# HBioquant/DiffBindFR

Measured on AMD Instinct MI355X. Metric: poses_per_sec, higher is better.
Workload: dtype f32

## Files before the change

### diffbindfr_amd/csrc/convz.hip

```cpp
#include <cstdio>
#include <cstdlib>
#include <type_traits>

#include "common.h"

typedef float f32x4 __attribute__((ext_vector_type(4)));
typedef float f32x2 __attribute__((ext_vector_type(2)));
typedef _Float16 f16x8 __attribute__((ext_vector_type(8)));
typedef _Float16 f16x4 __attribute__((ext_vector_type(4)));
typedef _Float16 f16x2 __attribute__((ext_vector_type(2)));
typedef unsigned u32x4 __attribute__((ext_vector_type(4)));
typedef unsigned u32x2 __attribute__((ext_vector_type(2)));

#define CH_TILE_BYTES 9280
#define CH_TAIL_OFF 8192
#define CH_BIAS_OFF 9216

#define CZ_VSTRIDE 2064
#define CZ_CB (8 * CZ_VSTRIDE)
#define CZ_NCB 2
#define CZ_TILE (CZ_NCB * CZ_CB)
#define CZ_KPB 1
#define CZ_BUF (CZ_KPB * CZ_TILE)
#define CZ_ZBYTES (2 * CZ_BUF)
#define CZ_NHL 2
#define CZ_WAVE_FLOATS (32 * 12 + 32 + 32 + 32 + 32 + 32 + CZ_MAXSEG * 16 + 24 * 64 + CZ_NHL * 256)
#ifndef CZ_PRIO
#define CZ_PRIO 1
#endif
#if CZ_PRIO
#define CZ_SETPRIO(x) __builtin_amdgcn_s_setprio(x)
#else
#define CZ_SETPRIO(x)
#endif
#ifndef CZ_FETCH_AT
#define CZ_FETCH_AT 4
#endif
#ifndef CZ_PF_KT
#define CZ_PF_KT 7
#endif
#define CZ_ZSCALE (-20)

__device__ __forceinline__ void cz_split2(float x0, float x1, unsigned& hi, unsigned& lo) {
  const f16x2 h = __builtin_convertvector((f32x2){x0, x1}, f16x2);
  const f16x2 l = __builtin_convertvector((f32x2){x0 - (float)h[0], x1 - (float)h[1]}, f16x2);
  hi = __builtin_bit_cast(unsigned, h);
  lo = __builtin_bit_cast(unsigned, l);
}
__device__ __forceinline__ float cz_wave_max(float v) {
#pragma unroll
  for (int o = 1; o < 64; o <<= 1) v = fmaxf(v, __shfl_xor(v, o));
  return v;
}

__device__ __forceinline__ int cz_lane_here() {
  int l = __builtin_amdgcn_mbcnt_hi(~0u, __builtin_amdgcn_mbcnt_lo(~0u, 0u));
  asm volatile("" : "+v"(l));
  return l;
}

template <int I, int N, typename F>
__device__ __forceinline__ void cz_static_for(F&& f) {
  if constexpr (I < N) { f(std::integral_constant<int, I>{}); cz_static_for<I + 1, N>(f); }
}

template <int NW, int ABL = 0>
__global__ __launch_bounds__(64 * NW, 2) void k_convz(ConvZArgs a) {
  constexpr int KT = 9;
  extern __shared__ __attribute__((aligned(16))) float lds[];
  const int tid = threadIdx.x, lane = tid & 63, wave = __builtin_amdgcn_readfirstlane(tid >> 6);
  const int n = lane & 15, g = lane >> 4;
  char* zb = reinterpret_cast<char*>(lds);
  float* wl = lds + CZ_ZBYTES / 4 + wave * CZ_WAVE_FLOATS;
  float* w_sh = wl;
  float* w_sa = wl + 32 * 12;
  float* w_ua = w_sa + 32;
  int* w_row = reinterpret_cast<int*>(w_ua + 32);
  int* w_seg = w_row + 32;
  int* w_first = w_seg + 32;
  unsigned* w_mask = reinterpret_cast<unsigned*>(w_first + 32);
  float* w_xs = reinterpret_cast<float*>(w_mask + CZ_MAXSEG * 16);
  u32x4* w_hl = reinterpret_cast<u32x4*>(w_xs + 24 * 64);
  int* b_nseg = reinterpret_cast<int*>(lds + CZ_ZBYTES / 4 + NW * CZ_WAVE_FLOATS);
  int* b_col_edge = b_nseg + NW;
  float* b_col_inv = reinterpret_cast<float*>(b_col_edge + 16 * CZ_NCB);
  unsigned* b_cdesc = reinterpret_cast<unsigned*>(b_col_inv + 16 * CZ_NCB);

  int tr_n = 0;
  auto stamp = [&](int tag) {
    if constexpr ((ABL & 128) != 0) {
      if (a.dbg && blockIdx.x == 0 && lane == 0 && tr_n < 1000) {
        unsigned long long* t = reinterpret_cast<unsigned long long*>(a.dbg) + wave * 1024;
        t[tr_n++] = (__builtin_amdgcn_s_memtime() << 8) | (unsigned)tag;
      }
    }
  };
  int nch[4] = {0, 0, 0, 0}, nu[4] = {0, 0, 0, 0};
#pragma unroll
  for (int c = 0; c < 4; ++c)
    if (c < a.n_conv) {
      const ConvZDesc& d = a.c[c];
      nch[c] = min(*d.n_chunks, d.max_chunks);
      nu[c] = (nch[c] + NW - 1) / NW;
    }
  const int N = nu[0] + nu[1] + nu[2] + nu[3];
  for (int unit = blockIdx.x; unit < N; unit += gridDim.x) {
    int c = 0, ul = unit;
    if (ul >= nu[0]) { ul -= nu[0]; c = 1; if (ul >= nu[1]) { ul -= nu[1]; c = 2; if (ul >= nu[2]) { ul -= nu[2]; c = 3; } } }
    const ConvZDesc& d = a.c[c];
    const ConvZ& W = d.w;
    const int E = min(*d.n_edges, d.max_edges);
    const int ch = ul * NW + wave;
    int es = 0, len = 0, gidx = 0;
    if (ch < nch[c]) {
      es = d.chunk_es[ch];
      const int gl = d.chunk_gl[ch];
      gidx = gl >> 6;
      len = min(min(gl & 63, 32), max(E - es, 0));
    }
    __syncthreads();
    if (tid < CZ_MAXCT * 16) b_cdesc[tid] = tid < (W.ct0[W.n_io - 1] + W.nct[W.n_io - 1]) * 16 ? W.cdesc[tid] : 0u;
    if (unit != (int)blockIdx.x) tr_n = 1000;
    stamp(1);
    const int sl = lane & 31;
    const bool have = len > 0;
    const int e_sl = have ? es + min(sl, len - 1) : 0;
    int tgt_l = 0, gth_l = 0;
    if (have) { tgt_l = d.tgt[e_sl]; gth_l = d.gth[e_sl]; }
    const int tgt_prev = __shfl_up(tgt_l, 1);
    const bool is_first = lane < 32 && sl < len && (sl == 0 || tgt_l != tgt_prev);
    const unsigned long long bal = __ballot(is_first);
    const unsigned firsts = (unsigned)bal;
    const int nseg = min(__popc(firsts), CZ_MAXSEG);
    const int seg_l = (sl < len) ? __popc(firsts & (0xffffffffu >> (31 - sl))) - 1 : -1;
    if (lane < 32) {
      w_row[sl] = gth_l * d.ldx;
      w_seg[sl] = seg_l;
      if (is_first) w_first[seg_l] = sl;
      const float* sp = d.sh + (size_t)e_sl * SH_LD;
#pragma unroll
      for (int k = 0; k < 9; ++k) w_sh[sl * 12 + k] = have ? sp[k] : 0.f;
      w_sh[sl * 12 + 9] = w_sh[sl * 12 + 10] = w_sh[sl * 12 + 11] = 0.f;
    }
    if (lane == 0) b_nseg[wave] = nseg;
    float xmx = 0.f, smx = 0.f;
    if (have) {
      if (d.xmax) xmx = d.xmax[gidx];
      else {
        const float* xr = d.x + (size_t)gth_l * d.ldx;
        const int d4 = d.ldx >> 2;
        for (int j = lane >> 5; j < d4; j += 2) {
          const f32x4 v = *reinterpret_cast<const f32x4*>(xr + 4 * j);
          xmx = fmaxf(fmaxf(xmx, fmaxf(fabsf(v[0]), fabsf(v[1]))), fmaxf(fabsf(v[2]), fabsf(v[3])));
        }
      }
      if (lane < 32) {
        const float* sp = d.sh + (size_t)e_sl * SH_LD;
#pragma unroll
        for (int k = 0; k < 9; ++k) smx = fmaxf(smx, fabsf(sp[k]));
      }
    }
    xmx = cz_wave_max(xmx); smx = cz_wave_max(smx);
    int ey = 0;
    if (xmx > 0.f && smx > 0.f) ey = max(-100, min(100, 13 - __builtin_amdgcn_frexp_expf(xmx) - __builtin_amdgcn_frexp_expf(smx)));
    ey = __builtin_amdgcn_readfirstlane(ey);
    const float sY = __builtin_amdgcn_ldexpf(1.f, ey);

    stamp(2);
    u32x4 Hh[CZ_NKT][2];
    int eh = 0;
    {
      const __amdgpu_buffer_rsrc_t rW1 = __builtin_amdgcn_make_buffer_rsrc((void*)W.W1h, 0, KT * CH_TILE_BYTES, 0x00020000);
      u32x4 Ah[2][2][4];
      u32x4 Atc[2];
#pragma unroll
      for (int et = 0; et < 2; ++et) {
        const int slot = 16 * et + n;
        const int e = have ? es + min(slot, len - 1) : 0;
        const float* r0 = d.emb + (size_t)e * NS;
        const float* r1 = d.tab1 + (size_t)(have ? d.idx1[e] : 0) * d.ld1;
        const float* r2 = d.tab2 + (size_t)(have ? d.idx2[e] : 0) * d.ld2;
        f32x4 Ba[KT];
        float amx = 0.f;
#pragma unroll
        for (int s4 = 0; s4 < KT; ++s4) {
          const float* src = s4 < 3 ? r0 : s4 < 6 ? r1 : r2;
          Ba[s4] = have ? *reinterpret_cast<const f32x4*>(src + 16 * (s4 % 3) + 4 * g) : (f32x4){0.f, 0.f, 0.f, 0.f};
#pragma unroll
          for (int q = 0; q < 4; ++q) amx = fmaxf(amx, fabsf(Ba[s4][q]));
        }
        amx = fmaxf(amx, __shfl_xor(amx, 16));
        amx = fmaxf(amx, __shfl_xor(amx, 32));
        const int ja = max(-14, __builtin_amdgcn_frexp_expf(amx));
        const float sa = __builtin_amdgcn_ldexpf(1.f, 15 - ja);
        if (g == 0) { w_sa[slot] = sa; w_ua[slot] = __builtin_amdgcn_ldexpf(1.f, ja - 15); }
#pragma unroll
        for (int s4 = 0; s4 < KT; ++s4) {
          unsigned hi0, lo0, hi1, lo1;
          cz_split2(Ba[s4][0] * sa, Ba[s4][1] * sa, hi0, lo0);
          cz_split2(Ba[s4][2] * sa, Ba[s4][3] * sa, hi1, lo1);
          if (s4 < 8) {
            Ah[et][0][s4 >> 1][2 * (s4 & 1)] = hi0; Ah[et][0][s4 >> 1][2 * (s4 & 1) + 1] = hi1;
            Ah[et][1][s4 >> 1][2 * (s4 & 1)] = lo0; Ah[et][1][s4 >> 1][2 * (s4 & 1) + 1] = lo1;
          } else {
            Atc[et] = (u32x4){lo0, lo1, hi0, hi1};
          }
        }
      }
      __builtin_amdgcn_wave_barrier();
      f32x4 sar[2], uar[2];
#pragma unroll
      for (int et = 0; et < 2; ++et) {
        sar[et] = *reinterpret_cast<const f32x4*>(w_sa + 16 * et + 4 * g);
        uar[et] = *reinterpret_cast<const f32x4*>(w_ua + 16 * et + 4 * g);
      }
      float Hf[KT][2][4];
      float hmx = 0.f;
      const int vW = lane * 16;
      u32x4 F[3][2];
      auto ldF = [&](auto ic) {
        constexpr int i = decltype(ic)::value, m = i / 5, sx = i % 5;
        if constexpr (sx < 4) {
          F[i % 3][0] = __builtin_bit_cast(u32x4, __builtin_amdgcn_raw_buffer_load_b128(rW1, vW, m * CH_TILE_BYTES + sx * 1024, 0));
          F[i % 3][1] = __builtin_bit_cast(u32x4, __builtin_amdgcn_raw_buffer_load_b128(rW1, vW, m * CH_TILE_BYTES + (4 + sx) * 1024, 0));
        } else {
          F[i % 3][0] = __builtin_bit_cast(u32x4, __builtin_amdgcn_raw_buffer_load_b128(rW1, vW, m * CH_TILE_BYTES + CH_TAIL_OFF, 0));
          F[i % 3][1][0] = __builtin_amdgcn_raw_buffer_load_b32(rW1, n * 4, m * CH_TILE_BYTES + CH_BIAS_OFF, 0);
        }
      };
      ldF(std::integral_constant<int, 0>{});
      ldF(std::integral_constant<int, 1>{});
      f32x4 acc[2];
      cz_static_for<0, 5 * KT>([&](auto ic) {
        constexpr int i = decltype(ic)::value, m = i / 5, sx = i % 5;
        if constexpr (i + 2 < 5 * KT) ldF(std::integral_constant<int, (i + 2 < 5 * KT ? i + 2 : 0)>{});
        if constexpr (sx == 0) { acc[0] = (f32x4){0.f, 0.f, 0.f, 0.f}; acc[1] = (f32x4){0.f, 0.f, 0.f, 0.f}; }
        if constexpr (sx < 4) {
          const f16x8 whi = __builtin_bit_cast(f16x8, F[i % 3][0]), wlo = __builtin_bit_cast(f16x8, F[i % 3][1]);
#pragma unroll
          for (int et = 0; et < 2; ++et) {
            acc[et] = __builtin_amdgcn_mfma_f32_16x16x32_f16(__builtin_bit_cast(f16x8, Ah[et][1][sx]), whi, acc[et], 0, 0, 0);
            acc[et] = __builtin_amdgcn_mfma_f32_16x16x32_f16(__builtin_bit_cast(f16x8, Ah[et][0][sx]), wlo, acc[et], 0, 0, 0);
            acc[et] = __builtin_amdgcn_mfma_f32_16x16x32_f16(__builtin_bit_cast(f16x8, Ah[et][0][sx]), whi, acc[et], 0, 0, 0);
          }
        } else {
          const u32x4 wt = F[i % 3][0];
          const f16x8 wf = __builtin_bit_cast(f16x8, wt);
          const f16x8 wh = __builtin_bit_cast(f16x8, (u32x4){wt[0], wt[1], 0u, 0u});
          const float bias = __builtin_bit_cast(float, F[i % 3][1][0]);
          const float w1r = W.W1rinv ? W.W1rinv[16 * m + n] : 1.f;
#pragma unroll
          for (int et = 0; et < 2; ++et) {
            acc[et] = __builtin_amdgcn_mfma_f32_16x16x32_f16(__builtin_bit_cast(f16x8, Atc[et]), wf, acc[et], 0, 0, 0);
            acc[et] = __builtin_amdgcn_mfma_f32_16x16x32_f16(__builtin_bit_cast(f16x8, (u32x4){Atc[et][2], Atc[et][3], 0u, 0u}), wh, acc[et], 0, 0, 0);
          }
#pragma unroll
          for (int et = 0; et < 2; ++et)
#pragma unroll
            for (int q = 0; q < 4; ++q) {
              const float v = fmaxf(acc[et][q] + bias * sar[et][q], 0.f) * (uar[et][q] * w1r);
              Hf[m][et][q] = v;
              hmx = fmaxf(hmx, v);
            }
        }
      });
      if (!(ABL & 128) && a.dbg && unit == 0 && wave == 0) {
        const float k1i = __builtin_amdgcn_ldexpf(1.f, -W.k1);
#pragma unroll
        for (int m = 0; m < KT; ++m)
#pragma unroll
          for (int et = 0; et < 2; ++et)
#pragma unroll
            for (int q = 0; q < 4; ++q) a.dbg[(16 * et + 4 * g + q) * 144 + 16 * m + n] = Hf[m][et][q] * k1i;
      }
      hmx = cz_wave_max(hmx);
      eh = max(hmx > 0.f ? __builtin_amdgcn_frexp_expf(hmx) : W.k1, W.k1);
      eh = min(eh, W.k1 + 100);
      const float sH = __builtin_amdgcn_ldexpf(1.f, 15 - eh);
#pragma unroll
      for (int m = 0; m < KT; ++m) {
        unsigned h0, l0, h1, l1, h2, l2, h3, l3;
        cz_split2(Hf[m][0][0] * sH, Hf[m][0][1] * sH, h0, l0);
        cz_split2(Hf[m][0][2] * sH, Hf[m][0][3] * sH, h1, l1);
        cz_split2(Hf[m][1][0] * sH, Hf[m][1][1] * sH, h2, l2);
        cz_split2(Hf[m][1][2] * sH, Hf[m][1][3] * sH, h3, l3);
        Hh[m][0] = (u32x4){h0, h1, h2, h3};
        if (m < CZ_NHL) w_hl[m * 64 + lane] = (u32x4){l0, l1, l2, l3};
        else Hh[m][1] = (u32x4){l0, l1, l2, l3};
      }
    }
    const int ephi = 15 - eh + W.k1;
    {
      const _Float16 ph = (_Float16)__builtin_amdgcn_ldexpf(1.f, ephi);
      const unsigned short pb = __builtin_bit_cast(unsigned short, ph);
      u32x4 hb = {0u, 0u, 0u, 0u};
      if (n == 0) {
#pragma unroll
        for (int t = 0; t < 8; ++t) {
          const int slot = t < 4 ? 4 * g + t : 16 + 4 * g + (t - 4);
          if (slot < len) hb[t >> 1] |= (unsigned)pb << (16 * (t & 1));
        }
      }
      Hh[KT][0] = hb;
      Hh[KT][1] = (u32x4){0u, 0u, 0u, 0u};
    }
    stamp(3);
    {
      const int j = lane >> 4, gg = (lane >> 2) & 3, r = lane & 3, t0 = 2 * r;
      const int s0 = t0 < 4 ? 4 * gg + t0 : 16 + 4 * gg + (t0 - 4);
      w_mask[lane] = (w_seg[s0] == j ? 0x0000ffffu : 0u) | (w_seg[s0 + 1] == j ? 0xffff0000u : 0u);
    }
    __builtin_amdgcn_wave_barrier();
    __syncthreads();
    int cbase = 0, total = 0;
#pragma unroll
    for (int v = 0; v < NW; ++v) { const int c = b_nseg[v]; if (v < wave) cbase += c; total += c; }
    cbase = __builtin_amdgcn_readfirstlane(cbase); total = __builtin_amdgcn_readfirstlane(total);
    const int nseg_u = __builtin_amdgcn_readfirstlane(nseg);
    const int ncb = (total + 15) >> 4;
    const float col_inv = __builtin_amdgcn_ldexpf(1.f, -CZ_ZSCALE - ey - ephi);
    const float zs = __builtin_amdgcn_ldexpf(1.f, CZ_ZSCALE);
    if (ABL & 32) continue;
    for (int c = tid; c < 16 * CZ_NCB; c += 64 * NW) b_col_edge[c] = -1;
    __syncthreads();
    if (lane < nseg_u) {
      b_col_edge[cbase + lane] = es + w_first[lane];
      b_col_inv[cbase + lane] = col_inv;
    }
    char* za[CZ_MAXSEG];
    {
      char* zw0 = zb + (n & 7) * CZ_VSTRIDE + g * 512 + (n >> 3) * 256;
#pragma unroll
      for (int j = 0; j < CZ_MAXSEG; ++j) {
        const int col = cbase + j;
        za[j] = j < nseg_u ? zw0 + (col >> 4) * CZ_CB + (col & 15) * 16 : zw0 + CZ_CB + 15 * 16;
      }
    }
    long long n_mfma = 2 * KT * 14;
    for (int io = 0; io < W.n_io; ++io) {
      n_mfma += (long long)W.nct[io] * (3LL * CZ_NKT * CZ_MAXSEG + 9LL * ncb * (KT + (wave == 0)));
      f32x4 acc[3][CZ_NCB];
#pragma unroll
      for (int wt = 0; wt < 3; ++wt)
#pragma unroll
        for (int cb = 0; cb < CZ_NCB; ++cb) acc[wt][cb] = (f32x4){0.f, 0.f, 0.f, 0.f};
      const char* wbase = reinterpret_cast<const char*>(W.W2z) + (size_t)lane * 16;
      int gq = W.ct0[io] * CZ_NKT;
      const int gq_last = (W.ct0[io] + W.nct[io]) * CZ_NKT - 1;
      u32x4 Wf[2][3][2];
      auto fetchW = [&](auto par_c, int q, int share) {
        constexpr int par = decltype(par_c)::value;
        if ((ABL & 1) && q != W.ct0[io] * CZ_NKT) return;
        const char* p = wbase + ((size_t)q * 8 + share) * CZ_TILE_BYTES;
#pragma unroll
        for (int wt = 0; wt < 3; ++wt)
#pragma unroll
          for (int pc = 0; pc < 2; ++pc) Wf[par][wt][pc] = *reinterpret_cast<const u32x4*>(p + (wt * 2 + pc) * 1024);
      };
      u32x4 Ym[CZ_MAXSEG][2];
#pragma unroll
      for (int j = 0; j < CZ_MAXSEG; ++j) { Ym[j][0] = (u32x4){0u, 0u, 0u, 0u}; Ym[j][1] = (u32x4){0u, 0u, 0u, 0u}; }
      auto prefetch_x = [&](int ct) {
        if (nseg_u == 0 || (ABL & 16)) return;
        const int lane = __builtin_amdgcn_mbcnt_hi(~0u, __builtin_amdgcn_mbcnt_lo(~0u, 0u)), n = lane & 15, g = lane >> 4;
        const unsigned cd_n = b_cdesc[(W.ct0[io] + ct) * 16 + n];
        const bool vec = (__builtin_amdgcn_readfirstlane(cd_n) >> 12) & 1u;
        const int xo = cd_n & 0xfff;
        const unsigned lds0 = (unsigned)(size_t)(const void __attribute__((address_space(3)))*)w_xs;
#pragma unroll
        for (int t = 0; t < 8; ++t) {
          const float* xp = d.x + w_row[t < 4 ? 4 * g + t : 16 + 4 * g + (t - 4)] + xo;
          asm volatile("s_mov_b32 m0, %0\n\ts_nop 0\n\tglobal_load_lds_dword %1, off" ::"s"(__builtin_amdgcn_readfirstlane(lds0 + t * 256)), "v"(xp) : "memory");
          if (vec) {
            asm volatile("s_mov_b32 m0, %0\n\ts_nop 0\n\tglobal_load_lds_dword %1, off" ::"s"(__builtin_amdgcn_readfirstlane(lds0 + (8 + t) * 256)), "v"(xp + 1) : "memory");
            asm volatile("s_mov_b32 m0, %0\n\ts_nop 0\n\tglobal_load_lds_dword %1, off" ::"s"(__builtin_amdgcn_readfirstlane(lds0 + (16 + t) * 256)), "v"(xp + 2) : "memory");
          }
        }
      };
      auto wait_stage = [&](auto younger_c) {
        constexpr int y = decltype(younger_c)::value;
        static_assert(y == 0 || y == 6, "wait_stage: a fetch is six loads");
        __builtin_amdgcn_sched_barrier(0);
        if constexpr (y == 0) asm volatile("s_waitcnt vmcnt(0)" ::: "memory");
        else asm volatile("s_waitcnt vmcnt(6)" ::: "memory");
        __builtin_amdgcn_sched_barrier(0);
      };
      auto finish_Y = [&](int ct) {
        if (nseg_u == 0 || (ABL & 16)) return;
        const int lane = cz_lane_here(), n = lane & 15, g = lane >> 4;
        const unsigned cd_n = b_cdesc[(W.ct0[io] + ct) * 16 + n];
        const bool vec = (__builtin_amdgcn_readfirstlane(cd_n) >> 12) & 1u;
        const int so = (cd_n >> 16) & 15;
        const float yv = (cd_n >> 31) ? sY : 0.f;
        float y[8];
        if (!vec) {
          float xs[8], s0[8];
#pragma unroll
          for (int t = 0; t < 8; ++t) { xs[t] = w_xs[t * 64 + lane]; s0[t] = w_sh[(t < 4 ? 4 * g + t : 16 + 4 * g + (t - 4)) * 12 + so]; }
#pragma unroll
          for (int t = 0; t < 8; ++t) y[t] = xs[t] * s0[t] * yv;
        } else {
          float xs[8][3], s1[8][3];
#pragma unroll
          for (int t = 0; t < 8; ++t)
#pragma unroll
            for (int m = 0; m < 3; ++m) { xs[t][m] = w_xs[(8 * m + t) * 64 + lane]; s1[t][m] = w_sh[(t < 4 ? 4 * g + t : 16 + 4 * g + (t - 4)) * 12 + so + m]; }
#pragma unroll
          for (int t = 0; t < 8; ++t) y[t] = (xs[t][0] * s1[t][0] + xs[t][1] * s1[t][1] + xs[t][2] * s1[t][2]) * yv;
        }
        u32x4 Yh, Yl;
#pragma unroll
        for (int r = 0; r < 4; ++r) { unsigned hi, lo; cz_split2(y[2 * r], y[2 * r + 1], hi, lo); Yh[r] = hi; Yl[r] = lo; }
#pragma unroll
        for (int j = 0; j < CZ_MAXSEG; ++j) {
          const u32x4 mk = *reinterpret_cast<const u32x4*>(w_mask + (j * 4 + g) * 4);
          Ym[j][0] = Yh & mk; Ym[j][1] = Yl & mk;
        }
      };
#define YM(j, p) __builtin_bit_cast(f16x8, Ym[j][p])
#define MF(a, b, c) __builtin_amdgcn_mfma_f32_16x16x32_f16(a, b, c, 0, 0, 0)
#define SL __builtin_amdgcn_sched_barrier(0)
      auto load_hl = [&](auto kt_c) -> u32x4 {
        constexpr int kt = decltype(kt_c)::value;
        if constexpr (kt < CZ_NHL) {
          return w_hl[kt * 64 + cz_lane_here()];
        } else
          return Hh[kt][1];
      };
      auto stepA = [&](auto kt_c, auto buf_c) {
        constexpr int kt = decltype(kt_c)::value, boff = decltype(buf_c)::value * CZ_BUF;
        if (ABL & 4) return;
        const f32x4 zero = {0.f, 0.f, 0.f, 0.f};
        const f16x8 hh = __builtin_bit_cast(f16x8, Hh[kt][0]), hl = __builtin_bit_cast(f16x8, load_hl(kt_c));
        f32x4 z[CZ_MAXSEG];
#pragma unroll
        for (int j = 0; j < CZ_MAXSEG; ++j) z[j] = MF(YM(j, 0), hl, zero);
#pragma unroll
        for (int j = 0; j < CZ_MAXSEG; ++j) z[j] = MF(YM(j, 1), hh, z[j]);
#pragma unroll
        for (int j = 0; j < CZ_MAXSEG; ++j) z[j] = MF(YM(j, 0), hh, z[j]);
#pragma unroll
        for (int j = 0; j < CZ_MAXSEG; ++j) *reinterpret_cast<f32x4*>(za[j] + boff) = z[j];
      };
      auto cut = [&](const f32x4 (&zf)[2], u32x4& zh, u32x4& zl, auto r_c) {
        constexpr int r = decltype(r_c)::value;
        unsigned hi, lo;
        cz_split2(zf[r >> 1][2 * (r & 1)] * zs, zf[r >> 1][2 * (r & 1) + 1] * zs, hi, lo);
        zh[r] = hi; zl[r] = lo;
      };
      using K0 = std::integral_constant<int, 0>; using K1 = std::integral_constant<int, 1>;
      using K2 = std::integral_constant<int, 2>; using K3 = std::integral_constant<int, 3>;
      auto tile = [&](auto kt_c, auto ncb_c) {
        constexpr int kt = decltype(kt_c)::value, NCBV = decltype(ncb_c)::value;
        constexpr int boffA = ((kt + 1) & 1) * CZ_BUF;
        if constexpr (CZ_FETCH_AT == 0) fetchW(std::integral_constant<int, (kt + 1) & 1>{}, min(gq + 1, gq_last), kt + 1 == KT ? 0 : wave);
        const char* zr = zb + (kt & 1) * CZ_BUF + wave * CZ_VSTRIDE + g * 512 + n * 16;
        f32x4 zf0[2], zf1[2];
        zf0[0] = *reinterpret_cast<const f32x4*>(zr); zf0[1] = *reinterpret_cast<const f32x4*>(zr + 256);
        const f32x4 zero = {0.f, 0.f, 0.f, 0.f};
        const f16x8 hh = __builtin_bit_cast(f16x8, Hh[kt + 1][0]), hl = __builtin_bit_cast(f16x8, load_hl(std::integral_constant<int, kt + 1>{}));
        u32x4 p0h, p0l, p1h, p1l;
        f32x4 z0, z1, z2, z3;
        if constexpr ((ABL & 4) != 0) {
          z0 = z1 = z2 = z3 = zero;
          cut(zf0, p0h, p0l, K0{}); cut(zf0, p0h, p0l, K1{}); cut(zf0, p0h, p0l, K2{}); cut(zf0, p0h, p0l, K3{});
        } else {
        CZ_SETPRIO(3);
        SL;
        z0 = MF(YM(0, 0), hl, zero); SL;
        z1 = MF(YM(1, 0), hl, zero); SL;
        z2 = MF(YM(2, 0), hl, zero); SL;
        z3 = MF(YM(3, 0), hl, zero); SL;
        if constexpr (CZ_FETCH_AT == 4) { fetchW(std::integral_constant<int, (kt + 1) & 1>{}, min(gq + 1, gq_last), kt + 1 == KT ? 0 : wave); SL; }
        z0 = MF(YM(0, 1), hh, z0); cut(zf0, p0h, p0l, K0{}); SL;
        z1 = MF(YM(1, 1), hh, z1); SL;
        z2 = MF(YM(2, 1), hh, z2); cut(zf0, p0h, p0l, K1{}); SL;
        z3 = MF(YM(3, 1), hh, z3); SL;
        if constexpr (CZ_FETCH_AT == 8) { fetchW(std::integral_constant<int, (kt + 1) & 1>{}, min(gq + 1, gq_last), kt + 1 == KT ? 0 : wave); SL; }
        CZ_SETPRIO(2);
        z0 = MF(YM(0, 0), hh, z0); cut(zf0, p0h, p0l, K2{}); SL;
        z1 = MF(YM(1, 0), hh, z1); SL;
        z2 = MF(YM(2, 0), hh, z2); cut(zf0, p0h, p0l, K3{}); SL;
        z3 = MF(YM(3, 0), hh, z3); SL;
        if constexpr (CZ_FETCH_AT == 12) { fetchW(std::integral_constant<int, (kt + 1) & 1>{}, min(gq + 1, gq_last), kt + 1 == KT ? 0 : wave); SL; }
        }
        if constexpr ((ABL & 4) != 0 && CZ_FETCH_AT != 0) fetchW(std::integral_constant<int, (kt + 1) & 1>{}, min(gq + 1, gq_last), kt + 1 == KT ? 0 : wave);
#define WFR(wt, pc) __builtin_bit_cast(f16x8, Wf[kt & 1][wt][pc])
        if constexpr ((ABL & 8) != 0) {
          if constexpr (!(ABL & 4)) { *reinterpret_cast<f32x4*>(za[0] + boffA) = z0; *reinterpret_cast<f32x4*>(za[1] + boffA) = z1; *reinterpret_cast<f32x4*>(za[2] + boffA) = z2; *reinterpret_cast<f32x4*>(za[3] + boffA) = z3; }
          asm volatile("" :: "v"(p0h), "v"(p0l));
        } else {
          const f16x8 zh = __builtin_bit_cast(f16x8, p0h), zl = __builtin_bit_cast(f16x8, p0l);
          if constexpr (NCBV > 1) { zf1[0] = *reinterpret_cast<const f32x4*>(zr + CZ_CB); zf1[1] = *reinterpret_cast<const f32x4*>(zr + CZ_CB + 256); }
          acc[0][0] = MF(WFR(0, 0), zl, acc[0][0]); *reinterpret_cast<f32x4*>(za[0] + boffA) = z0; SL;
          acc[1][0] = MF(WFR(1, 0), zl, acc[1][0]); *reinterpret_cast<f32x4*>(za[1] + boffA) = z1; SL;
          acc[2][0] = MF(WFR(2, 0), zl, acc[2][0]); *reinterpret_cast<f32x4*>(za[2] + boffA) = z2; SL;
          acc[0][0] = MF(WFR(0, 1), zh, acc[0][0]); *reinterpret_cast<f32x4*>(za[3] + boffA) = z3; SL;
          CZ_SETPRIO(1);
          acc[1][0] = MF(WFR(1, 1), zh, acc[1][0]); if constexpr (NCBV > 1) cut(zf1, p1h, p1l, K0{}); SL;
          acc[2][0] = MF(WFR(2, 1), zh, acc[2][0]); if constexpr (NCBV > 1) cut(zf1, p1h, p1l, K1{}); SL;
          acc[0][0] = MF(WFR(0, 0), zh, acc[0][0]); if constexpr (NCBV > 1) cut(zf1, p1h, p1l, K2{}); SL;
          acc[1][0] = MF(WFR(1, 0), zh, acc[1][0]); if constexpr (NCBV > 1) cut(zf1, p1h, p1l, K3{}); SL;
          acc[2][0] = MF(WFR(2, 0), zh, acc[2][0]); SL;
        }
        if constexpr (NCBV > 1 && !(ABL & 8)) {
          const f16x8 zh = __builtin_bit_cast(f16x8, p1h), zl = __builtin_bit_cast(f16x8, p1l);
          acc[0][1] = MF(WFR(0, 0), zl, acc[0][1]); SL;
          acc[1][1] = MF(WFR(1, 0), zl, acc[1][1]); SL;
          acc[2][1] = MF(WFR(2, 0), zl, acc[2][1]); SL;
          CZ_SETPRIO(0);
          acc[0][1] = MF(WFR(0, 1), zh, acc[0][1]); SL;
          acc[1][1] = MF(WFR(1, 1), zh, acc[1][1]); SL;
          acc[2][1] = MF(WFR(2, 1), zh, acc[2][1]); SL;
          acc[0][1] = MF(WFR(0, 0), zh, acc[0][1]); SL;
          acc[1][1] = MF(WFR(1, 0), zh, acc[1][1]); SL;
          acc[2][1] = MF(WFR(2, 0), zh, acc[2][1]); SL;
        }
      };
      auto tile9 = [&](int ct) {
        constexpr int kt = KT;
        fetchW(K0{}, min(gq + 1, gq_last), wave);
        wait_stage(std::integral_constant<int, 6>{});
        if (wave == 0 && !(ABL & 8)) {
          const int lane = cz_lane_here(), n = lane & 15, g = lane >> 4;
          const char* zr = zb + (kt & 1) * CZ_BUF + g * 512 + n * 16;
#pragma unroll
          for (int cb = 0; cb < CZ_NCB; ++cb)
            if (cb < ncb) {
              f32x4 zf[2];
              zf[0] = *reinterpret_cast<const f32x4*>(zr + cb * CZ_CB); zf[1] = *reinterpret_cast<const f32x4*>(zr + cb * CZ_CB + 256);
              u32x4 ph, pl;
              cut(zf, ph, pl, K0{}); cut(zf, ph, pl, K1{}); cut(zf, ph, pl, K2{}); cut(zf, ph, pl, K3{});
              const f16x8 zh = __builtin_bit_cast(f16x8, ph), zl = __builtin_bit_cast(f16x8, pl);
#pragma unroll
              for (int wt = 0; wt < 3; ++wt) {
                acc[wt][cb] = MF(WFR(wt, 0), zl, acc[wt][cb]);
                acc[wt][cb] = MF(WFR(wt, 1), zh, acc[wt][cb]);
                acc[wt][cb] = MF(WFR(wt, 0), zh, acc[wt][cb]);
              }
            }
        }
        if (ct + 1 < W.nct[io]) { finish_Y(ct + 1); stepA(K0{}, K0{}); }
      };
#undef WFR
      prefetch_x(0);
      wait_stage(K0{});
      auto run_tiles = [&](auto ncb_c) {
        fetchW(K0{}, gq, wave);
        finish_Y(0);
        stepA(K0{}, K0{});
        __syncthreads();
        for (int ct = 0; ct < W.nct[io]; ++ct) {
          cz_static_for<0, CZ_NKT>([&](auto kt_c) {
            constexpr int kt = decltype(kt_c)::value;
            stamp(10);
            if constexpr (kt < KT) {
              tile(kt_c, ncb_c);
              if constexpr (kt == CZ_PF_KT) if (ct + 1 < W.nct[io]) prefetch_x(ct + 1);
            } else
              tile9(ct);
            stamp(12);
            ++gq;
            if (!(ABL & 2)) __syncthreads();
            stamp(13);
          });
        }
      };
      if (ncb > 1) run_tiles(K2{}); else run_tiles(K1{});
#undef YM
#undef MF
#undef SL
      float* red = reinterpret_cast<float*>(zb) + wave * (12 * CZ_NCB * 64);
#pragma unroll
      for (int wt = 0; wt < 3; ++wt)
#pragma unroll
        for (int cb = 0; cb < CZ_NCB; ++cb)
#pragma unroll
          for (int q = 0; q < 4; ++q) red[((wt * CZ_NCB + cb) * 4 + q) * 64 + lane] = acc[wt][cb][q];
      __syncthreads();
      for (int idx = tid; idx < 16 * ncb * 48; idx += 64 * NW) {
        const int col = idx / 48, w = idx - 48 * col;
        const int e = b_col_edge[col];
        if (e >= 0) {
          const int r = w & 15;
          const float* rp = reinterpret_cast<const float*>(zb) + (((w >> 4) * CZ_NCB + (col >> 4)) * 4 + (r & 3)) * 64 + 16 * (r >> 2) + (col & 15);
          float s = 0.f;
#pragma unroll
          for (int v = 0; v < NW; ++v) s += rp[v * (12 * CZ_NCB * 64)];
          d.msg[(size_t)e * d.D_out + W.out_off[io] + w] = s * b_col_inv[col] * W.rowinv[io * 48 + w];
        }
      }
      __syncthreads();
    }
    if (a.executed && lane == 0) atomicAdd(a.executed, 16384.0 * (double)n_mfma);
  }
}

__global__ void k_convz_useful(ConvZArgs a) {
  for (int c = 0; c < a.n_conv; ++c) {
    const ConvZDesc& d = a.c[c];
    const ConvZ& W = d.w;
    const int nch = min(*d.n_chunks, d.max_chunks), E = min(*d.n_edges, d.max_edges);
    double useful = 0.0, bytes = 0.0;
    for (int ch = blockIdx.x * blockDim.x + threadIdx.x; ch < nch; ch += gridDim.x * blockDim.x) {
      const int es = d.chunk_es[ch], len = min(min(d.chunk_gl[ch] & 63, 32), max(E - es, 0));
      int nseg = 0;
      for (int i = 0; i < len; ++i) nseg += (i == 0 || d.tgt[es + i] != d.tgt[es + i - 1]);
      nseg = min(nseg, CZ_MAXSEG);
      double u = 144.0 * 144.0 * len;
      for (int io = 0; io < W.n_io; ++io) u += (double)W.nc_valid[io] * 145.0 * ((double)len + 48.0 * nseg);
      useful += 6.0 * u;
      bytes += 4.0 * 48.0 * W.n_io * nseg;
    }
    if (useful > 0.0) { atomicAdd(a.executed + 1, useful); atomicAdd(a.executed + 2, bytes); }
  }
}

size_t convz_lds_bytes() { return CZ_ZBYTES + 8 * CZ_WAVE_FLOATS * sizeof(float) + (8 + 2 * 16 * CZ_NCB + CZ_MAXCT * 16) * sizeof(int); }

void launch_convz(const ConvZArgs& a0, hipStream_t st) {
  constexpr int NW = 8;
  ConvZArgs a = a0;
  static float* dbg_dev = nullptr;
  static const char* dbg_file = getenv("DBFR_CONVZ_DEBUG");
  if (dbg_file && !dbg_dev) {
    if (hipMalloc(&dbg_dev, 8 * 1024 * 8) != hipSuccess || hipMemset(dbg_dev, 0, 8 * 1024 * 8) != hipSuccess) dbg_dev = nullptr;
    else atexit([] {
      std::vector<float> h(8 * 1024 * 2);
      if (hipDeviceSynchronize() == hipSuccess && hipMemcpy(h.data(), dbg_dev, h.size() * 4, hipMemcpyDeviceToHost) == hipSuccess)
        if (FILE* f = fopen(getenv("DBFR_CONVZ_DEBUG"), "wb")) { fwrite(h.data(), 4, h.size(), f); fclose(f); }
    });
  }
  a.dbg = dbg_dev;
  const size_t lds = convz_lds_bytes();
#define V(x) { if (dbfr_launch_check(hipFuncSetAttribute(reinterpret_cast<const void*>(&k_convz<NW, x>), hipFuncAttributeMaxDynamicSharedMemorySize, (int)lds), "k_convz: hipFuncSetAttribute(MaxDynamicSharedMemorySize)")) return; \
               hipLaunchKernelGGL((k_convz<NW, x>), dim3(dbfr_current_cu_count()), dim3(64 * NW), lds, st, a); return; }
#ifdef DBFR_DEV_VARIANTS
  static int abl = getenv("DBFR_CONVZ_ABL") ? atoi(getenv("DBFR_CONVZ_ABL")) : 0;
  if (abl == 1) V(1) if (abl == 2) V(2) if (abl == 4) V(4) if (abl == 8) V(8) if (abl == 16) V(16) if (abl == 32) V(32) if (abl == 12) V(12) if (abl == 5) V(5) if (abl == 64) V(64) if (abl == 128) V(128)
#endif
  if (a.executed) hipLaunchKernelGGL(k_convz_useful, dim3(64), dim3(256), 0, st, a);
  V(0)
#undef V
}
```

Baseline: 524.4.

## Hoist and overlap per-chunk gathers in convz prologue with next-chunk prefetch

Restructures the per-unit prologue of the convz kernel. The next unit's chunk descriptors are prefetched through constant-address loads, and all embedding and table gathers plus spherical-harmonic loads are issued up front in one batch. The first column tile's x-gather into LDS is launched early, before the H-stage MFMA loop, and the cdesc LDS store is deferred. The debug dump is moved behind a compile-time flag, and sched barriers are added in the W1 loop. The aim is to hide global-memory latency in the prologue, at the cost of more live registers (Ba for both edge tiles) and possible occupancy pressure.

```diff
diff --git a/diffbindfr_amd/csrc/convz.hip b/diffbindfr_amd/csrc/convz.hip
--- a/diffbindfr_amd/csrc/convz.hip
+++ b/diffbindfr_amd/csrc/convz.hip
@@ -87,9 +87,10 @@
   unsigned* b_cdesc = reinterpret_cast<unsigned*>(b_col_inv + 16 * CZ_NCB);
 
   int tr_n = 0;
+  bool tr_on = false;
   auto stamp = [&](int tag) {
     if constexpr ((ABL & 128) != 0) {
-      if (a.dbg && blockIdx.x == 0 && lane == 0 && tr_n < 1000) {
+      if (a.dbg && tr_on && lane == 0 && tr_n < 1000) {
         unsigned long long* t = reinterpret_cast<unsigned long long*>(a.dbg) + wave * 1024;
         t[tr_n++] = (__builtin_amdgcn_s_memtime() << 8) | (unsigned)tag;
       }
@@ -104,60 +105,124 @@
       nu[c] = (nch[c] + NW - 1) / NW;
     }
   const int N = nu[0] + nu[1] + nu[2] + nu[3];
+  typedef const int __attribute__((address_space(4))) * cz_cptr;
+  auto chunk_entry = [&](int u, int& es_, int& gl_) {
+    es_ = 0; gl_ = 0;
+    if (u < N) {
+      int c = 0, ul = u;
+      if (ul >= nu[0]) { ul -= nu[0]; c = 1; if (ul >= nu[1]) { ul -= nu[1]; c = 2; if (ul >= nu[2]) { ul -= nu[2]; c = 3; } } }
+      const int ch = ul * NW + wave;
+      if (ch < nch[c]) { es_ = ((cz_cptr)a.c[c].chunk_es)[ch]; gl_ = ((cz_cptr)a.c[c].chunk_gl)[ch]; }
+    }
+  };
+  int nx_es, nx_gl;
+  chunk_entry(blockIdx.x, nx_es, nx_gl);
   for (int unit = blockIdx.x; unit < N; unit += gridDim.x) {
     int c = 0, ul = unit;
     if (ul >= nu[0]) { ul -= nu[0]; c = 1; if (ul >= nu[1]) { ul -= nu[1]; c = 2; if (ul >= nu[2]) { ul -= nu[2]; c = 3; } } }
     const ConvZDesc& d = a.c[c];
     const ConvZ& W = d.w;
-    const int E = min(*d.n_edges, d.max_edges);
-    const int ch = ul * NW + wave;
-    int es = 0, len = 0, gidx = 0;
-    if (ch < nch[c]) {
-      es = d.chunk_es[ch];
-      const int gl = d.chunk_gl[ch];
-      gidx = gl >> 6;
-      len = min(min(gl & 63, 32), max(E - es, 0));
-    }
+    const int E = min(*(cz_cptr)d.n_edges, d.max_edges);
+    const int es = nx_es, gl = nx_gl;
+    const int gidx = gl >> 6;
+    const int len = min(min(gl & 63, 32), max(E - es, 0));
+    chunk_entry(unit + gridDim.x, nx_es, nx_gl);
     __syncthreads();
-    if (tid < CZ_MAXCT * 16) b_cdesc[tid] = tid < (W.ct0[W.n_io - 1] + W.nct[W.n_io - 1]) * 16 ? W.cdesc[tid] : 0u;
-    if (unit != (int)blockIdx.x) tr_n = 1000;
+    const int ncd = (W.ct0[W.n_io - 1] + W.nct[W.n_io - 1]) * 16;
+    const unsigned cdv = W.cdesc[min(tid, max(ncd - 1, 0))];
+    tr_on = blockIdx.x == 0 && unit == (int)gridDim.x;
     stamp(1);
-    const int sl = lane & 31;
+    const int pl = cz_lane_here(), pn = pl & 15, pg = pl >> 4;
+    const int sl = pl & 31;
     const bool have = len > 0;
     const int e_sl = have ? es + min(sl, len - 1) : 0;
     int tgt_l = 0, gth_l = 0;
-    if (have) { tgt_l = d.tgt[e_sl]; gth_l = d.gth[e_sl]; }
+    float shv[9] = {0.f, 0.f, 0.f, 0.f, 0.f, 0.f, 0.f, 0.f, 0.f};
+    float xmx = 0.f, smx = 0.f;
+    unsigned cd0 = 0u;
+    f32x4 Ba[2][KT];
+#pragma unroll
+    for (int et = 0; et < 2; ++et)
+#pragma unroll
+      for (int s4 = 0; s4 < KT; ++s4) Ba[et][s4] = (f32x4){0.f, 0.f, 0.f, 0.f};
+    if (have) {
+      const int e0 = es + min(pn, len - 1), e1 = es + min(16 + pn, len - 1);
+      const int i10 = d.idx1[e0], i11 = d.idx1[e1], i20 = d.idx2[e0], i21 = d.idx2[e1];
+      tgt_l = d.tgt[e_sl]; gth_l = d.gth[e_sl];
+      const float* sp = d.sh + (size_t)e_sl * SH_LD;
+#pragma unroll
+      for (int k = 0; k < 9; ++k) shv[k] = sp[k];
+      if (W.nct[0] > 0) cd0 = W.cdesc[W.ct0[0] * 16 + pn];
+      if (d.xmax) xmx = d.xmax[gidx];
+      const float* r00 = d.emb + (size_t)e0 * NS + 4 * pg;
+      const float* r01 = d.emb + (size_t)e1 * NS + 4 * pg;
+#pragma unroll
+      for (int s4 = 0; s4 < 3; ++s4) {
+        Ba[0][s4] = *reinterpret_cast<const f32x4*>(r00 + 16 * s4);
+        Ba[1][s4] = *reinterpret_cast<const f32x4*>(r01 + 16 * s4);
+      }
+      const float* r10 = d.tab1 + (size_t)i10 * d.ld1 + 4 * pg;
+      const float* r11 = d.tab1 + (size_t)i11 * d.ld1 + 4 * pg;
+      const float* r20 = d.tab2 + (size_t)i20 * d.ld2 + 4 * pg;
+      const float* r21 = d.tab2 + (size_t)i21 * d.ld2 + 4 * pg;
+#pragma unroll
+      for (int s4 = 0; s4 < 3; ++s4) {
+        Ba[0][3 + s4] = *reinterpret_cast<const f32x4*>(r10 + 16 * s4);
+        Ba[0][6 + s4] = *reinterpret_cast<const f32x4*>(r20 + 16 * s4);
+      }
+#pragma unroll
+      for (int s4 = 0; s4 < 3; ++s4) {
+        Ba[1][3 + s4] = *reinterpret_cast<const f32x4*>(r11 + 16 * s4);
+        Ba[1][6 + s4] = *reinterpret_cast<const f32x4*>(r21 + 16 * s4);
+      }
+    }
     const int tgt_prev = __shfl_up(tgt_l, 1);
-    const bool is_first = lane < 32 && sl < len && (sl == 0 || tgt_l != tgt_prev);
+    const bool is_first = pl < 32 && sl < len && (sl == 0 || tgt_l != tgt_prev);
     const unsigned long long bal = __ballot(is_first);
     const unsigned firsts = (unsigned)bal;
     const int nseg = min(__popc(firsts), CZ_MAXSEG);
     const int seg_l = (sl < len) ? __popc(firsts & (0xffffffffu >> (31 - sl))) - 1 : -1;
-    if (lane < 32) {
+    if (pl < 32) {
       w_row[sl] = gth_l * d.ldx;
       w_seg[sl] = seg_l;
       if (is_first) w_first[seg_l] = sl;
-      const float* sp = d.sh + (size_t)e_sl * SH_LD;
-#pragma unroll
-      for (int k = 0; k < 9; ++k) w_sh[sl * 12 + k] = have ? sp[k] : 0.f;
+#pragma unroll
+      for (int k = 0; k < 9; ++k) w_sh[sl * 12 + k] = shv[k];
       w_sh[sl * 12 + 9] = w_sh[sl * 12 + 10] = w_sh[sl * 12 + 11] = 0.f;
     }
     if (lane == 0) b_nseg[wave] = nseg;
-    float xmx = 0.f, smx = 0.f;
+    const int nseg_u = __builtin_amdgcn_readfirstlane(nseg);
+    auto gather_x = [&](auto&& cd_of) {
+      if (nseg_u == 0 || (ABL & 16)) return;
+      const int lane = __builtin_amdgcn_mbcnt_hi(~0u, __builtin_amdgcn_mbcnt_lo(~0u, 0u)), n = lane & 15, g = lane >> 4;
+      const unsigned cd_n = cd_of(n);
+      const bool vec = (__builtin_amdgcn_readfirstlane(cd_n) >> 12) & 1u;
+      const int xo = cd_n & 0xfff;
+      const unsigned lds0 = (unsigned)(size_t)(const void __attribute__((address_space(3)))*)w_xs;
+#pragma unroll
+      for (int t = 0; t < 8; ++t) {
+        const float* xp = d.x + w_row[t < 4 ? 4 * g + t : 16 + 4 * g + (t - 4)] + xo;
+        asm volatile("s_mov_b32 m0, %0\n\ts_nop 0\n\tglobal_load_lds_dword %1, off" ::"s"(__builtin_amdgcn_readfirstlane(lds0 + t * 256)), "v"(xp) : "memory");
+        if (vec) {
+          asm volatile("s_mov_b32 m0, %0\n\ts_nop 0\n\tglobal_load_lds_dword %1, off" ::"s"(__builtin_amdgcn_readfirstlane(lds0 + (8 + t) * 256)), "v"(xp + 1) : "memory");
+          asm volatile("s_mov_b32 m0, %0\n\ts_nop 0\n\tglobal_load_lds_dword %1, off" ::"s"(__builtin_amdgcn_readfirstlane(lds0 + (16 + t) * 256)), "v"(xp + 2) : "memory");
+        }
+      }
+    };
+    __builtin_amdgcn_wave_barrier();
+    if (W.nct[0] > 0) gather_x([&](int) { return cd0; });
     if (have) {
-      if (d.xmax) xmx = d.xmax[gidx];
-      else {
+      if (!d.xmax) {
         const float* xr = d.x + (size_t)gth_l * d.ldx;
         const int d4 = d.ldx >> 2;
-        for (int j = lane >> 5; j < d4; j += 2) {
+        for (int j = pl >> 5; j < d4; j += 2) {
           const f32x4 v = *reinterpret_cast<const f32x4*>(xr + 4 * j);
           xmx = fmaxf(fmaxf(xmx, fmaxf(fabsf(v[0]), fabsf(v[1]))), fmaxf(fabsf(v[2]), fabsf(v[3])));
         }
       }
-      if (lane < 32) {
-        const float* sp = d.sh + (size_t)e_sl * SH_LD;
-#pragma unroll
-        for (int k = 0; k < 9; ++k) smx = fmaxf(smx, fabsf(sp[k]));
+      if (pl < 32) {
+#pragma unroll
+        for (int k = 0; k < 9; ++k) smx = fmaxf(smx, fabsf(shv[k]));
       }
     }
     xmx = cz_wave_max(xmx); smx = cz_wave_max(smx);
@@ -175,30 +240,22 @@
       u32x4 Atc[2];
 #pragma unroll
       for (int et = 0; et < 2; ++et) {
-        const int slot = 16 * et + n;
-        const int e = have ? es + min(slot, len - 1) : 0;
-        const float* r0 = d.emb + (size_t)e * NS;
-        const float* r1 = d.tab1 + (size_t)(have ? d.idx1[e] : 0) * d.ld1;
-        const float* r2 = d.tab2 + (size_t)(have ? d.idx2[e] : 0) * d.ld2;
-        f32x4 Ba[KT];
+        const int slot = 16 * et + pn;
         float amx = 0.f;
 #pragma unroll
-        for (int s4 = 0; s4 < KT; ++s4) {
-          const float* src = s4 < 3 ? r0 : s4 < 6 ? r1 : r2;
-          Ba[s4] = have ? *reinterpret_cast<const f32x4*>(src + 16 * (s4 % 3) + 4 * g) : (f32x4){0.f, 0.f, 0.f, 0.f};
-#pragma unroll
-          for (int q = 0; q < 4; ++q) amx = fmaxf(amx, fabsf(Ba[s4][q]));
-        }
+        for (int s4 = 0; s4 < KT; ++s4)
+#pragma unroll
+          for (int q = 0; q < 4; ++q) amx = fmaxf(amx, fabsf(Ba[et][s4][q]));
         amx = fmaxf(amx, __shfl_xor(amx, 16));
         amx = fmaxf(amx, __shfl_xor(amx, 32));
         const int ja = max(-14, __builtin_amdgcn_frexp_expf(amx));
         const float sa = __builtin_amdgcn_ldexpf(1.f, 15 - ja);
-        if (g == 0) { w_sa[slot] = sa; w_ua[slot] = __builtin_amdgcn_ldexpf(1.f, ja - 15); }
+        if (pg == 0) { w_sa[slot] = sa; w_ua[slot] = __builtin_amdgcn_ldexpf(1.f, ja - 15); }
 #pragma unroll
         for (int s4 = 0; s4 < KT; ++s4) {
           unsigned hi0, lo0, hi1, lo1;
-          cz_split2(Ba[s4][0] * sa, Ba[s4][1] * sa, hi0, lo0);
-          cz_split2(Ba[s4][2] * sa, Ba[s4][3] * sa, hi1, lo1);
+          cz_split2(Ba[et][s4][0] * sa, Ba[et][s4][1] * sa, hi0, lo0);
+          cz_split2(Ba[et][s4][2] * sa, Ba[et][s4][3] * sa, hi1, lo1);
           if (s4 < 8) {
             Ah[et][0][s4 >> 1][2 * (s4 & 1)] = hi0; Ah[et][0][s4 >> 1][2 * (s4 & 1) + 1] = hi1;
             Ah[et][1][s4 >> 1][2 * (s4 & 1)] = lo0; Ah[et][1][s4 >> 1][2 * (s4 & 1) + 1] = lo1;
@@ -207,16 +264,19 @@
           }
         }
       }
+      if (tid < CZ_MAXCT * 16) b_cdesc[tid] = tid < ncd ? cdv : 0u;
+      stamp(4);
       __builtin_amdgcn_wave_barrier();
+      const int hl = cz_lane_here(), hn = hl & 15, hg = hl >> 4;
       f32x4 sar[2], uar[2];
 #pragma unroll
       for (int et = 0; et < 2; ++et) {
-        sar[et] = *reinterpret_cast<const f32x4*>(w_sa + 16 * et + 4 * g);
-        uar[et] = *reinterpret_cast<const f32x4*>(w_ua + 16 * et + 4 * g);
+        sar[et] = *reinterpret_cast<const f32x4*>(w_sa + 16 * et + 4 * hg);
+        uar[et] = *reinterpret_cast<const f32x4*>(w_ua + 16 * et + 4 * hg);
       }
       float Hf[KT][2][4];
       float hmx = 0.f;
-      const int vW = lane * 16;
+      const int vW = hl * 16;
       u32x4 F[3][2];
       auto ldF = [&](auto ic) {
         constexpr int i = decltype(ic)::value, m = i / 5, sx = i % 5;
@@ -225,14 +285,17 @@
           F[i % 3][1] = __builtin_bit_cast(u32x4, __builtin_amdgcn_raw_buffer_load_b128(rW1, vW, m * CH_TILE_BYTES + (4 + sx) * 1024, 0));
         } else {
           F[i % 3][0] = __builtin_bit_cast(u32x4, __builtin_amdgcn_raw_buffer_load_b128(rW1, vW, m * CH_TILE_BYTES + CH_TAIL_OFF, 0));
-          F[i % 3][1][0] = __builtin_amdgcn_raw_buffer_load_b32(rW1, n * 4, m * CH_TILE_BYTES + CH_BIAS_OFF, 0);
-        }
-      };
+          F[i % 3][1][0] = __builtin_amdgcn_raw_buffer_load_b32(rW1, hn * 4, m * CH_TILE_BYTES + CH_BIAS_OFF, 0);
+        }
+      };
+      const float* w1ri = W.W1rinv;
+      asm volatile("" : "+s"(w1ri));
       ldF(std::integral_constant<int, 0>{});
       ldF(std::integral_constant<int, 1>{});
       f32x4 acc[2];
       cz_static_for<0, 5 * KT>([&](auto ic) {
         constexpr int i = decltype(ic)::value, m = i / 5, sx = i % 5;
+        __builtin_amdgcn_sched_barrier(0);
         if constexpr (i + 2 < 5 * KT) ldF(std::integral_constant<int, (i + 2 < 5 * KT ? i + 2 : 0)>{});
         if constexpr (sx == 0) { acc[0] = (f32x4){0.f, 0.f, 0.f, 0.f}; acc[1] = (f32x4){0.f, 0.f, 0.f, 0.f}; }
         if constexpr (sx < 4) {
@@ -248,7 +311,7 @@
           const f16x8 wf = __builtin_bit_cast(f16x8, wt);
           const f16x8 wh = __builtin_bit_cast(f16x8, (u32x4){wt[0], wt[1], 0u, 0u});
           const float bias = __builtin_bit_cast(float, F[i % 3][1][0]);
-          const float w1r = W.W1rinv ? W.W1rinv[16 * m + n] : 1.f;
+          const float w1r = w1ri ? w1ri[16 * m + hn] : 1.f;
 #pragma unroll
           for (int et = 0; et < 2; ++et) {
             acc[et] = __builtin_amdgcn_mfma_f32_16x16x32_f16(__builtin_bit_cast(f16x8, Atc[et]), wf, acc[et], 0, 0, 0);
@@ -264,7 +327,8 @@
             }
         }
       });
-      if (!(ABL & 128) && a.dbg && unit == 0 && wave == 0) {
+      stamp(5);
+      if constexpr ((ABL & 256) != 0) if (a.dbg && unit == 0 && wave == 0) {
         const float k1i = __builtin_amdgcn_ldexpf(1.f, -W.k1);
 #pragma unroll
         for (int m = 0; m < KT; ++m)
@@ -274,6 +338,7 @@
             for (int q = 0; q < 4; ++q) a.dbg[(16 * et + 4 * g + q) * 144 + 16 * m + n] = Hf[m][et][q] * k1i;
       }
       hmx = cz_wave_max(hmx);
+      const int cl = cz_lane_here();
       eh = max(hmx > 0.f ? __builtin_amdgcn_frexp_expf(hmx) : W.k1, W.k1);
       eh = min(eh, W.k1 + 100);
       const float sH = __builtin_amdgcn_ldexpf(1.f, 15 - eh);
@@ -285,7 +350,7 @@
         cz_split2(Hf[m][1][0] * sH, Hf[m][1][1] * sH, h2, l2);
         cz_split2(Hf[m][1][2] * sH, Hf[m][1][3] * sH, h3, l3);
         Hh[m][0] = (u32x4){h0, h1, h2, h3};
-        if (m < CZ_NHL) w_hl[m * 64 + lane] = (u32x4){l0, l1, l2, l3};
+        if (m < CZ_NHL) w_hl[m * 64 + cl] = (u32x4){l0, l1, l2, l3};
         else Hh[m][1] = (u32x4){l0, l1, l2, l3};
       }
     }
@@ -293,8 +358,9 @@
     {
       const _Float16 ph = (_Float16)__builtin_amdgcn_ldexpf(1.f, ephi);
       const unsigned short pb = __builtin_bit_cast(unsigned short, ph);
+      const int bl = cz_lane_here(), g = bl >> 4;
       u32x4 hb = {0u, 0u, 0u, 0u};
-      if (n == 0) {
+      if ((bl & 15) == 0) {
 #pragma unroll
         for (int t = 0; t < 8; ++t) {
           const int slot = t < 4 ? 4 * g + t : 16 + 4 * g + (t - 4);
@@ -306,7 +372,7 @@
     }
     stamp(3);
     {
-      const int j = lane >> 4, gg = (lane >> 2) & 3, r = lane & 3, t0 = 2 * r;
+      const int lane = cz_lane_here(), j = lane >> 4, gg = (lane >> 2) & 3, r = lane & 3, t0 = 2 * r;
       const int s0 = t0 < 4 ? 4 * gg + t0 : 16 + 4 * gg + (t0 - 4);
       w_mask[lane] = (w_seg[s0] == j ? 0x0000ffffu : 0u) | (w_seg[s0 + 1] == j ? 0xffff0000u : 0u);
     }
@@ -316,10 +382,10 @@
 #pragma unroll
     for (int v = 0; v < NW; ++v) { const int c = b_nseg[v]; if (v < wave) cbase += c; total += c; }
     cbase = __builtin_amdgcn_readfirstlane(cbase); total = __builtin_amdgcn_readfirstlane(total);
-    const int nseg_u = __builtin_amdgcn_readfirstlane(nseg);
     const int ncb = (total + 15) >> 4;
     const float col_inv = __builtin_amdgcn_ldexpf(1.f, -CZ_ZSCALE - ey - ephi);
     const float zs = __builtin_amdgcn_ldexpf(1.f, CZ_ZSCALE);
+    stamp(6);
     if (ABL & 32) continue;
     for (int c = tid; c < 16 * CZ_NCB; c += 64 * NW) b_col_edge[c] = -1;
     __syncthreads();
@@ -360,23 +426,7 @@
       u32x4 Ym[CZ_MAXSEG][2];
 #pragma unroll
       for (int j = 0; j < CZ_MAXSEG; ++j) { Ym[j][0] = (u32x4){0u, 0u, 0u, 0u}; Ym[j][1] = (u32x4){0u, 0u, 0u, 0u}; }
-      auto prefetch_x = [&](int ct) {
-        if (nseg_u == 0 || (ABL & 16)) return;
-        const int lane = __builtin_amdgcn_mbcnt_hi(~0u, __builtin_amdgcn_mbcnt_lo(~0u, 0u)), n = lane & 15, g = lane >> 4;
-        const unsigned cd_n = b_cdesc[(W.ct0[io] + ct) * 16 + n];
-        const bool vec = (__builtin_amdgcn_readfirstlane(cd_n) >> 12) & 1u;
-        const int xo = cd_n & 0xfff;
-        const unsigned lds0 = (unsigned)(size_t)(const void __attribute__((address_space(3)))*)w_xs;
-#pragma unroll
-        for (int t = 0; t < 8; ++t) {
-          const float* xp = d.x + w_row[t < 4 ? 4 * g + t : 16 + 4 * g + (t - 4)] + xo;
-          asm volatile("s_mov_b32 m0, %0\n\ts_nop 0\n\tglobal_load_lds_dword %1, off" ::"s"(__builtin_amdgcn_readfirstlane(lds0 + t * 256)), "v"(xp) : "memory");
-          if (vec) {
-            asm volatile("s_mov_b32 m0, %0\n\ts_nop 0\n\tglobal_load_lds_dword %1, off" ::"s"(__builtin_amdgcn_readfirstlane(lds0 + (8 + t) * 256)), "v"(xp + 1) : "memory");
-            asm volatile("s_mov_b32 m0, %0\n\ts_nop 0\n\tglobal_load_lds_dword %1, off" ::"s"(__builtin_amdgcn_readfirstlane(lds0 + (16 + t) * 256)), "v"(xp + 2) : "memory");
-          }
-        }
-      };
+      auto prefetch_x = [&](int ct) { gather_x([&](int n) { return b_cdesc[(W.ct0[io] + ct) * 16 + n]; }); };
       auto wait_stage = [&](auto younger_c) {
         constexpr int y = decltype(younger_c)::value;
         static_assert(y == 0 || y == 6, "wait_stage: a fetch is six loads");
@@ -543,7 +593,7 @@
         if (ct + 1 < W.nct[io]) { finish_Y(ct + 1); stepA(K0{}, K0{}); }
       };
 #undef WFR
-      prefetch_x(0);
+      if (io > 0) prefetch_x(0);
       wait_stage(K0{});
       auto run_tiles = [&](auto ncb_c) {
         fetchW(K0{}, gq, wave);
@@ -637,7 +687,7 @@
                hipLaunchKernelGGL((k_convz<NW, x>), dim3(dbfr_current_cu_count()), dim3(64 * NW), lds, st, a); return; }
 #ifdef DBFR_DEV_VARIANTS
   static int abl = getenv("DBFR_CONVZ_ABL") ? atoi(getenv("DBFR_CONVZ_ABL")) : 0;
-  if (abl == 1) V(1) if (abl == 2) V(2) if (abl == 4) V(4) if (abl == 8) V(8) if (abl == 16) V(16) if (abl == 32) V(32) if (abl == 12) V(12) if (abl == 5) V(5) if (abl == 64) V(64) if (abl == 128) V(128)
+  if (abl == 1) V(1) if (abl == 2) V(2) if (abl == 4) V(4) if (abl == 8) V(8) if (abl == 16) V(16) if (abl == 32) V(32) if (abl == 12) V(12) if (abl == 5) V(5) if (abl == 64) V(64) if (abl == 128) V(128) if (abl == 256) V(256)
 #endif
   if (a.executed) hipLaunchKernelGGL(k_convz_useful, dim3(64), dim3(256), 0, st, a);
   V(0)
```

Result: no change. 520.5 (-0.7%).
